# theislab/dca

Hardware: NVIDIA H100
Metric: cells/sec (ZINB AE epoch, device-timed) (higher is better)
Workload: dtype bf16-gemm/f32-acc/f32-loss

## Files before the change

dca_b200/csrc/gene_gemm_tc.cu:

```cuda
#include "engine.h"
#include "tc_common.cuh"

namespace dca {
namespace tc {
int g_gg_profile = 0;
int g_head_bwd_banded = 1;
int g_head_bwd_stagger = 1300;
namespace gg {

constexpr int kThreads = 256;
constexpr uint32_t kZBytes = 128 * 128 * 2;
constexpr uint32_t kWBytes = 64 * 128 * 2;
constexpr uint32_t kHBytes = 128 * 64 * 2;
constexpr uint32_t kOutBytes = 128 * 64 * 4;
constexpr uint32_t kOnesBytes = 16 * 128;
constexpr int kMaxGb = 4;
constexpr int kMaxSlots = 16;

static_assert(kWBytes == kHBytes, "the two item kinds of the banded launch share one stage shape");
template <bool DO_A, bool DO_B, bool BANDED>
constexpr int stages() { return DO_A && DO_B && !BANDED ? 2 : 3; }
template <bool DO_A, bool DO_B, bool BANDED>
constexpr uint32_t stage_bytes() { return BANDED ? kZBytes + kWBytes : kZBytes + (DO_B ? kWBytes : 0) + (DO_A ? kHBytes : 0); }
template <bool DO_A, bool DO_B, bool COLSUM, bool BANDED>
constexpr uint32_t smem_bytes() {
  return stages<DO_A, DO_B, BANDED>() * stage_bytes<DO_A, DO_B, BANDED>() + (DO_A ? kOutBytes : 0) + (COLSUM ? kOnesBytes : 0) + 1024;
}

struct BandItem { int kind, head, gr, gb0, ng, cb0, ncb; };

__host__ __device__ inline BandItem band_item(int k, int n_gb, int n_cb, int gpr, int ranges) {
  const int per_head = n_gb + ranges * n_cb, full_band = gpr + n_cb;
  BandItem it;
  it.head = k / per_head; k -= it.head * per_head;
  it.gr = min(k / full_band, ranges - 1); k -= it.gr * full_band;
  const int gb0 = it.gr * gpr, ng = min(n_gb, gb0 + gpr) - gb0, m = min(ng, n_cb);
  int idx;
  if (k < 2 * m) { it.kind = k & 1; idx = k >> 1; }
  else { it.kind = ng > n_cb ? 0 : 1; idx = k - m; }
  if (it.kind == 0) { it.gb0 = gb0 + idx; it.ng = 1; it.cb0 = 0; it.ncb = n_cb; }
  else { it.gb0 = gb0; it.ng = ng; it.cb0 = idx; it.ncb = 1; }
  return it;
}

struct Params {
  int B, G, n_heads;
  int n_cb, n_gb;
  int gb_per_item, cb_per_item;
  int gene_ranges, cell_splits;
  int total_items;
  int stagger;
  float* db[3];
  float* part; int64_t part_stride;
  const int32_t* rows; const __nv_bfloat16* zsrc; int64_t ldz;
};

__device__ __forceinline__ void cp_async_16(uint32_t smem_dst, const void* src, uint32_t src_bytes) {
  asm volatile("cp.async.cg.shared.global [%0], [%1], 16, %2;" ::"r"(smem_dst), "l"(src), "r"(src_bytes) : "memory");
}
__device__ __forceinline__ void cp_async_commit() { asm volatile("cp.async.commit_group;" ::: "memory"); }
template <int N>
__device__ __forceinline__ void cp_async_wait() { asm volatile("cp.async.wait_group %0;" ::"n"(N) : "memory"); }

template <bool DO_A, bool DO_B, bool COLSUM, bool WK, int MAXG, bool BANDED>
__global__ void __launch_bounds__(kThreads, 1)
gene_gemm_kernel(const __grid_constant__ CUtensorMap map_z0, const __grid_constant__ CUtensorMap map_z1,
                 const __grid_constant__ CUtensorMap map_z2, const __grid_constant__ CUtensorMap map_h,
                 const __grid_constant__ CUtensorMap map_w0, const __grid_constant__ CUtensorMap map_w1,
                 const __grid_constant__ CUtensorMap map_w2, const __grid_constant__ CUtensorMap map_dw0, const __grid_constant__ CUtensorMap map_dw1,
                 const __grid_constant__ CUtensorMap map_dw2, const int dw_transposed, const Params p) {
  static_assert(!BANDED || (DO_A && DO_B && MAXG == 1), "banded items hold one gene block of (a) accumulators");
  constexpr int kStages = stages<DO_A, DO_B, BANDED>();
  constexpr uint32_t kStage = stage_bytes<DO_A, DO_B, BANDED>();
  constexpr uint32_t kHOff = kZBytes + (DO_B && !BANDED ? kWBytes : 0);
  extern __shared__ __align__(1024) uint8_t smem_raw[];
  uint8_t* smem = smem_raw + ((1024u - (smem_u32(smem_raw) & 1023u)) & 1023u);
  uint8_t* s_st = smem;
  float* s_o = reinterpret_cast<float*>(s_st + kStages * kStage);
  uint8_t* s_ones = reinterpret_cast<uint8_t*>(s_o) + (DO_A ? kOutBytes : 0);
  __shared__ uint64_t full[kStages];

  if (threadIdx.x == 0) {
    for (int i = 0; i < kStages; ++i) mbar_init(&full[i], 1);
    fence_barrier_init();
  }
  if (COLSUM) {
    for (int i = threadIdx.x; i < (int)kOnesBytes / 4; i += kThreads) reinterpret_cast<uint32_t*>(s_ones)[i] = 0x3F803F80u;
    fence_proxy_async_smem();
  }
  __syncthreads();

  const int wg = threadIdx.x >> 7, w = (threadIdx.x >> 5) & 3, l = threadIdx.x & 31;
  const int frow = 16 * w + (l >> 2), fcol = 2 * (l & 3);

  auto stage_begin = [&]() {
    if (threadIdx.x == 0) bulk_wait_read<0>();
    __syncthreads();
  };
  auto stage_end = [&](const CUtensorMap* m, int c0, int c1) {
    fence_proxy_async_smem();
    __syncthreads();
    if (threadIdx.x == 0) { tma_reduce_add_2d(m, c0, c1, s_o); bulk_commit(); }
  };

  uint32_t T0 = 0;
  const bool gather = p.rows != nullptr;
  const int g_rh = threadIdx.x >> 3, g_c = threadIdx.x & 7, g_h = g_rh & 1, g_r0 = g_rh >> 1;
  const uint32_t g_dst = g_h * (kZBytes / 2) + g_r0 * 128 + ((g_c ^ (g_r0 & 7)) << 4);
  int src_row[8];
  if constexpr (BANDED) {
    if (p.stagger > 0 && blockIdx.x < p.total_items) {
      const BandItem it = band_item(blockIdx.x, p.n_gb, p.n_cb, p.gb_per_item, p.gene_ranges);
      const long long wait = (long long)(it.kind ? it.cb0 : it.gb0 - it.gr * p.gb_per_item) * p.stagger;
      if (threadIdx.x == 0) {
        const long long c0 = clock64();
        while (clock64() - c0 < wait) __nanosleep(100);
      }
      __syncthreads();
    }
  }
  for (int item = blockIdx.x; item < p.total_items; item += gridDim.x) {
    int head, gr, gb0, ng, cb0, ncb;
    bool ia = DO_A, ib = DO_B;
    if constexpr (BANDED) {
      const BandItem it = band_item(item, p.n_gb, p.n_cb, p.gb_per_item, p.gene_ranges);
      head = it.head; gr = it.gr; gb0 = it.gb0; ng = it.ng; cb0 = it.cb0; ncb = it.ncb;
      ia = it.kind == 0; ib = !ia;
    } else {
      const int cs = item % p.cell_splits, r = item / p.cell_splits;
      gr = r % p.gene_ranges; head = r / p.gene_ranges;
      gb0 = gr * p.gb_per_item; ng = min(p.n_gb, gb0 + p.gb_per_item) - gb0;
      cb0 = cs * p.cb_per_item; ncb = min(p.n_cb, cb0 + p.cb_per_item) - cb0;
    }
    const int n_tiles = ng * ncb;
    const CUtensorMap* mz = head == 0 ? &map_z0 : (head == 1 ? &map_z1 : &map_z2);
    const CUtensorMap* mw = head == 0 ? &map_w0 : (head == 1 ? &map_w1 : &map_w2);
    const CUtensorMap* mdw = head == 0 ? &map_dw0 : (head == 1 ? &map_dw1 : &map_dw2);

    auto issue = [&](int t) {
      const int st = (T0 + t) % kStages;
      const int cb = cb0 + t / ng, gb = gb0 + t % ng;
      uint8_t* dst = s_st + st * kStage;
      mbar_expect_tx(&full[st], gather ? kStage - kZBytes : kStage);
      if (!gather) {
        tma_load_2d(dst, mz, gb * 128, cb * 128, &full[st]);
        tma_load_2d(dst + kZBytes / 2, mz, gb * 128 + 64, cb * 128, &full[st]);
      }
      if (DO_B && ib) {
        if (WK) {
          tma_load_2d(dst + kZBytes, mw, gb * 128, 0, &full[st]);
          tma_load_2d(dst + kZBytes + kWBytes / 2, mw, gb * 128 + 64, 0, &full[st]);
        } else {
          tma_load_2d(dst + kZBytes, mw, 0, gb * 128, &full[st]);
        }
      }
      if (DO_A && ia) tma_load_2d(dst + kHOff, &map_h, 0, cb * 128, &full[st]);
    };
    auto load_rows = [&](int t) {
      const int cb = cb0 + t / ng;
#pragma unroll
      for (int i = 0; i < 8; ++i) {
        const int r = cb * 128 + g_r0 + 16 * i;
        src_row[i] = r < p.B ? __ldg(p.rows + r) : -1;
      }
    };
    auto copy_rows = [&](int t) {
      const int st = (T0 + t) % kStages, g0 = (gb0 + t % ng) * 128 + g_h * 64 + g_c * 8;
      const uint32_t gbytes = g0 < p.G ? (uint32_t)min(16, 2 * (p.G - g0)) : 0u;
      const uint32_t dst = smem_u32(s_st + st * kStage) + g_dst;
#pragma unroll
      for (int i = 0; i < 8; ++i) {
        const bool ok = src_row[i] >= 0 && gbytes != 0;
        cp_async_16(dst + i * 2048, ok ? p.zsrc + (int64_t)src_row[i] * p.ldz + g0 : p.zsrc, ok ? gbytes : 0u);
      }
      if (t + 1 < n_tiles) load_rows(t + 1);
    };
    if (gather) load_rows(0);
    for (int t = 0; t < kStages - 1; ++t) {
      if (t < n_tiles) {
        if (threadIdx.x == 0) issue(t);
        if (gather) copy_rows(t);
      }
      if (gather) cp_async_commit();
    }

    float acc_b[DO_B ? 32 : 1];
    float acc_a[DO_A ? MAXG : 1][32];
    float acc_c[COLSUM ? MAXG : 1][8];
#pragma unroll
    for (int j = 0; j < (DO_A ? MAXG : 1); ++j)
#pragma unroll
      for (int i = 0; i < 32; ++i) acc_a[j][i] = 0.f;
#pragma unroll
    for (int j = 0; j < (COLSUM ? MAXG : 1); ++j)
#pragma unroll
      for (int i = 0; i < 8; ++i) acc_c[j][i] = 0.f;

    int t = 0;
    for (int cbi = 0; cbi < ncb; ++cbi) {
      const int cb = cb0 + cbi;
#pragma unroll
      for (int i = 0; i < (DO_B ? 32 : 1); ++i) acc_b[i] = 0.f;
#pragma unroll
      for (int jj = 0; jj < (DO_A ? MAXG : 1); ++jj)
      for (int j = jj; j < (DO_A && ia ? min(jj + 1, ng) : ng); ++j) {
        if (t + kStages - 1 < n_tiles) {
          if (threadIdx.x == 0) issue(t + kStages - 1);
          if (gather) copy_rows(t + kStages - 1);
        }
        if (gather) {
          cp_async_commit();
          cp_async_wait<kStages - 1>();
          fence_proxy_async_smem();
          __syncthreads();
        }
        const int st = (T0 + t) % kStages;
        mbar_wait(&full[st], ((T0 + t) / kStages) & 1);
        const uint32_t zb = smem_u32(s_st + st * kStage), wb = zb + kZBytes, hb = zb + kHOff;
        wgmma_fence();
        if constexpr (DO_B) {
          if (ib)
#pragma unroll
          for (int h = 0; h < 2; ++h)
#pragma unroll
            for (int k = 0; k < 4; ++k) {
              const uint64_t da = make_smem_desc(zb + h * (kZBytes / 2) + wg * 64 * 128 + k * 32, 0, 1024);
              if (WK) wgmma_m64n64k16<0, 0>(acc_b, da, make_smem_desc(wb + h * (kWBytes / 2) + k * 32, 0, 1024), 1u);
              else wgmma_m64n64k16<0, 1>(acc_b, da, make_smem_desc(wb + (h * 4 + k) * 2048, 0, 1024), 1u);
            }
        }
        if constexpr (DO_A) {
          if (ia)
#pragma unroll
          for (int k = 0; k < 8; ++k) {
            const uint64_t da = make_smem_desc(zb + wg * (kZBytes / 2) + k * 2048, 0, 1024);
            wgmma_m64n64k16<1, 1>(acc_a[jj], da, make_smem_desc(hb + k * 2048, 0, 1024), 1u);
            if constexpr (COLSUM) wgmma_m64n16k16<1, 0>(acc_c[jj], da, make_smem_desc(smem_u32(s_ones) + (k & 3) * 32, 0, 1024), 1u);
          }
        }
        wgmma_commit();
        wgmma_wait<0>();
        if constexpr (DO_B) acc_fence(acc_b);
        if constexpr (DO_A) {
#pragma unroll
          for (int jj2 = 0; jj2 < MAXG; ++jj2) acc_fence(acc_a[jj2]);
        }
        if constexpr (COLSUM) {
#pragma unroll
          for (int jj2 = 0; jj2 < MAXG; ++jj2) acc_fence(acc_c[jj2]);
        }
        __syncthreads();
        ++t;
      }
      if constexpr (DO_B) if (ib) {
        float* dst = p.part + (int64_t)(head * p.gene_ranges + gr) * p.part_stride + (int64_t)cb * 128 * 64;
#pragma unroll
        for (int i = 0; i < 32; i += 2) {
          const int row = wg * 64 + frow + 8 * ((i >> 1) & 1), col = 8 * (i >> 2) + fcol;
          *reinterpret_cast<float2*>(dst + row * 64 + col) = make_float2(acc_b[i], acc_b[i + 1]);
        }
      }
    }
    T0 += n_tiles;
    if (DO_A && ia) {
#pragma unroll
      for (int j = 0; j < MAXG; ++j) {
        if (j >= ng) break;
        const int gb = gb0 + j;
        stage_begin();
        if (dw_transposed) {
#pragma unroll
          for (int i = 0; i < 32; ++i) {
            const int g = wg * 64 + frow + 8 * ((i >> 1) & 1), f = 8 * (i >> 2) + fcol + (i & 1);
            s_o[f * 128 + g] = acc_a[j][i];
          }
          stage_end(mdw, gb * 128, 0);
        } else {
#pragma unroll
          for (int i = 0; i < 32; i += 2) {
            const int g = wg * 64 + frow + 8 * ((i >> 1) & 1), f = 8 * (i >> 2) + fcol;
            *reinterpret_cast<float2*>(s_o + g * 64 + f) = make_float2(acc_a[j][i], acc_a[j][i + 1]);
          }
          stage_end(mdw, 0, gb * 128);
        }
        if constexpr (COLSUM) {
          float* dbh = head == 0 ? p.db[0] : (head == 1 ? p.db[1] : p.db[2]);
          if ((l & 3) == 0 && dbh) {
            const int g = gb * 128 + wg * 64 + frow;
            if (g < p.G) atomicAdd(dbh + g, acc_c[j][0]);
            if (g + 8 < p.G) atomicAdd(dbh + g + 8, acc_c[j][2]);
          }
        }
      }
    }
  }
  if (threadIdx.x == 0) bulk_wait<0>();
}

__global__ void gene_gemm_reduce_kernel(const float* __restrict__ part, int slots, int64_t stride, float* __restrict__ out,
                                        int64_t n) {
  const int64_t i = ((int64_t)blockIdx.x * blockDim.x + threadIdx.x) * 4;
  if (i >= n) return;
  float4 acc = *reinterpret_cast<const float4*>(out + i);
  for (int sl = 0; sl < slots; ++sl) {
    const float4 v = __ldcs(reinterpret_cast<const float4*>(part + sl * stride + i));
    acc.x += v.x; acc.y += v.y; acc.z += v.z; acc.w += v.w;
  }
  *reinterpret_cast<float4*>(out + i) = acc;
}

void plan_a(Params& p, int n_heads, int sm_count) {
  int best_gpi = 1; long long best_cost = -1;
  for (int gpi = 1; gpi <= kMaxGb; ++gpi) {
    const long long items = (long long)cdiv(p.n_gb, gpi) * n_heads, rounds = (items + sm_count - 1) / sm_count;
    const long long cost = rounds * ((long long)gpi * p.n_cb + 2ll * gpi);
    if (best_cost < 0 || cost < best_cost) { best_cost = cost; best_gpi = gpi; }
  }
  p.gb_per_item = best_gpi; p.gene_ranges = cdiv(p.n_gb, best_gpi);
  p.cb_per_item = p.n_cb; p.cell_splits = 1;
  p.total_items = p.gene_ranges * n_heads;
}
void plan_b(Params& p, int n_heads, int sm_count) {
  p.cb_per_item = 1; p.cell_splits = p.n_cb;
  int gsplits = cdiv(4 * sm_count, p.n_cb * n_heads); if (gsplits < 1) gsplits = 1;
  if (gsplits > kMaxSlots / n_heads) gsplits = kMaxSlots / n_heads;
  if (gsplits > p.n_gb) gsplits = p.n_gb;
  while (gsplits > 1 && cdiv(p.n_gb, gsplits) < 4) --gsplits;
  p.gb_per_item = cdiv(p.n_gb, gsplits); p.gene_ranges = cdiv(p.n_gb, p.gb_per_item);
  p.total_items = p.gene_ranges * p.cell_splits * n_heads;
}
void plan_banded(Params& p, int n_heads, int sm_count, int* grid) {
  plan_b(p, n_heads, sm_count);
  p.total_items = n_heads * (p.n_gb + p.gene_ranges * p.n_cb);
  const int band = p.gb_per_item + p.n_cb;
  *grid = min(p.total_items, sm_count >= band ? sm_count / band * band : sm_count);
}

}

size_t gene_gemm_workspace_bytes(int B) { return sizeof(float) * (size_t)gg::kMaxSlots * cdiv(B, 128) * 128 * 64; }

int gene_gemm_tc(int mode, const __nv_bfloat16* const Z[3], int64_t ldz, const int32_t* rows, int B, int G, int n_heads,
                 const __nv_bfloat16* H, const __nv_bfloat16* const W[3], float* out_b, float* const dW[3], int64_t dW_ld,
                 int dW_transposed, float* const db[3], void* ws, size_t ws_bytes, int sm_count, cudaStream_t s) {
  using namespace gg;
  if (ldz % 8 != 0) { set_error("gene_gemm_tc: ldz must be a multiple of 8 (16-byte TMA stride)"); return DCA_ERR_BAD_ARG; }
  if (mode < 1 || mode > 3) { set_error("gene_gemm_tc: bad mode %d", mode); return DCA_ERR_BAD_ARG; }
  if (rows && (mode == 3 || n_heads != 1)) { set_error("gene_gemm_tc: row indices are for modes 1 and 2 (one Z)"); return DCA_ERR_BAD_ARG; }
  const bool do_a = mode & 2, do_b = mode & 1;
  if (do_b && (!ws || ws_bytes < gene_gemm_workspace_bytes(B))) { set_error("gene_gemm_tc: workspace too small"); return DCA_ERR_BAD_ARG; }
  CUtensorMap mz[3], mh, mw[3], mdw[3];
  for (int i = 0; i < 3; ++i) DCA_TRY(make_tensor_map_2d(&mz[i], Z[i < n_heads ? i : 0], 2, 1, (uint64_t)B, (uint64_t)G, (uint64_t)ldz, 128, 64, 1));
  mh = mz[0];
  for (int i = 0; i < 3; ++i) mw[i] = mdw[i] = mz[0];
  if (do_a) {
    DCA_TRY(make_tensor_map_2d(&mh, H, 2, 1, (uint64_t)B, 64, 64, 128, 64, 1));
    for (int i = 0; i < 3; ++i) {
      float* d = dW[i < n_heads ? i : 0];
      if (dW_transposed) DCA_TRY(make_tensor_map_2d(&mdw[i], d, 4, 0, 64, (uint64_t)G, (uint64_t)dW_ld, 64, 128, 0));
      else {
        if (dW_ld != 64) { set_error("gene_gemm_tc: non-transposed dW needs ld == 64"); return DCA_ERR_BAD_ARG; }
        DCA_TRY(make_tensor_map_2d(&mdw[i], d, 4, 0, (uint64_t)G, 64, 64, 128, 64, 0));
      }
    }
  }
  if (do_b) {
    for (int i = 0; i < 3; ++i) {
      const __nv_bfloat16* w = W[i < n_heads ? i : 0];
      if (mode == 3) DCA_TRY(make_tensor_map_2d(&mw[i], w, 2, 1, 64, (uint64_t)G, (uint64_t)G, 64, 64, 1));
      else DCA_TRY(make_tensor_map_2d(&mw[i], w, 2, 1, (uint64_t)G, 64, 64, 128, 64, 1));
    }
  }
  Params base{};
  base.B = B; base.G = G; base.n_heads = n_heads;
  base.n_cb = cdiv(B, 128); base.n_gb = cdiv(G, 128);
  for (int i = 0; i < 3; ++i) base.db[i] = db ? db[i] : nullptr;
  base.part = reinterpret_cast<float*>(ws); base.part_stride = (int64_t)base.n_cb * 128 * 64;
  base.rows = rows; base.zsrc = Z[0]; base.ldz = ldz;

#define DCA_GG_LAUNCH(P, GRID, A, Bb, Cc, WKk, MG, BND)                                                                \
  do {                                                                                                                 \
    static bool attr = false;                                                                                          \
    constexpr uint32_t sm = smem_bytes<A, Bb, Cc, BND>();                                                              \
    if (!attr) { DCA_CUDA_OK(cudaFuncSetAttribute(gene_gemm_kernel<A, Bb, Cc, WKk, MG, BND>, cudaFuncAttributeMaxDynamicSharedMemorySize, (int)sm)); attr = true; } \
    gene_gemm_kernel<A, Bb, Cc, WKk, MG, BND><<<GRID, kThreads, sm, s>>>(mz[0], mz[1], mz[2], mh, mw[0], mw[1], mw[2],  \
                                                                          mdw[0], mdw[1], mdw[2], dW_transposed, P);  \
    DCA_LAUNCH_CHECK();                                                                                                \
  } while (0)

  if (mode == 3 && g_head_bwd_banded) {
    Params p = base;
    int grid = 0;
    plan_banded(p, n_heads, sm_count, &grid);
    p.stagger = g_head_bwd_stagger;
    DCA_GG_LAUNCH(p, grid, true, true, true, true, 1, true);
    const int64_t n = (int64_t)B * 64;
    gene_gemm_reduce_kernel<<<(unsigned)cdiv(n / 4, 256), 256, 0, s>>>(p.part, p.gene_ranges * n_heads, p.part_stride, out_b, n);
    DCA_LAUNCH_CHECK();
    return DCA_OK;
  }
  if (do_a) {
    Params p = base;
    plan_a(p, n_heads, sm_count);
    const int grid = min(p.total_items, sm_count);
    if (mode == 3) DCA_GG_LAUNCH(p, grid, true, false, true, false, kMaxGb, false);
    else DCA_GG_LAUNCH(p, grid, true, false, false, false, kMaxGb, false);
  }
  if (do_b) {
    Params p = base;
    plan_b(p, n_heads, sm_count);
    const int grid = min(p.total_items, sm_count);
    if (mode == 3) DCA_GG_LAUNCH(p, grid, false, true, false, true, 1, false);
    else DCA_GG_LAUNCH(p, grid, false, true, false, false, 1, false);
    const int64_t n = (int64_t)B * 64;
    gene_gemm_reduce_kernel<<<(unsigned)cdiv(n / 4, 256), 256, 0, s>>>(p.part, p.gene_ranges * n_heads, p.part_stride, out_b, n);
    DCA_LAUNCH_CHECK();
  }
#undef DCA_GG_LAUNCH
  return DCA_OK;
}

}
}

using namespace dca;
extern "C" int dca_tc_gene_gemm_rows(int32_t mode, const void* Z0, const void* Z1, const void* Z2, int64_t ldz,
                                     const int32_t* rows, int32_t batch, int32_t genes, int32_t n_heads, const void* H,
                                     const void* W, float* out_b, float* dW0, float* dW1, float* dW2, int64_t dW_ld,
                                     int32_t dW_transposed, float* db0, float* db1, float* db2, void* stream, int32_t sm_count) {
  if (!Z0 || batch <= 0 || genes <= 0 || n_heads < 1 || n_heads > 3) { set_error("dca_tc_gene_gemm: bad argument"); return DCA_ERR_BAD_ARG; }
  int dev = 0, sms = 132;
  cudaGetDevice(&dev);
  cudaDeviceGetAttribute(&sms, cudaDevAttrMultiProcessorCount, dev);
  if (sm_count > 0 && sm_count < sms) sms = sm_count;
  const __nv_bfloat16* Z[3] = {(const __nv_bfloat16*)Z0, (const __nv_bfloat16*)Z1, (const __nv_bfloat16*)Z2};
  float* dW[3] = {dW0, dW1, dW2};
  float* db[3] = {db0, db1, db2};
  const __nv_bfloat16* Wp[3];
  for (int i = 0; i < 3; ++i) Wp[i] = (const __nv_bfloat16*)W + (mode == 3 ? (size_t)(i < n_heads ? i : 0) * 64 * genes : 0);
  cudaStream_t st = (cudaStream_t)stream;
  const size_t ws_bytes = tc::gene_gemm_workspace_bytes(batch);
  void* ws = nullptr;
  DCA_CUDA_OK(cudaMallocAsync(&ws, ws_bytes, st));
  const int rc = tc::gene_gemm_tc(mode, Z, ldz, rows, batch, genes, n_heads, (const __nv_bfloat16*)H, Wp, out_b, dW,
                                  dW_ld, dW_transposed, db, ws, ws_bytes, sms, st);
  DCA_CUDA_OK(cudaFreeAsync(ws, st));
  return rc;
}
extern "C" int dca_tc_gene_gemm_sms(int32_t mode, const void* Z0, const void* Z1, const void* Z2, int64_t ldz,
                                    int32_t batch, int32_t genes, int32_t n_heads, const void* H, const void* W, float* out_b,
                                    float* dW0, float* dW1, float* dW2, int64_t dW_ld, int32_t dW_transposed, float* db0,
                                    float* db1, float* db2, void* stream, int32_t sm_count) {
  return dca_tc_gene_gemm_rows(mode, Z0, Z1, Z2, ldz, nullptr, batch, genes, n_heads, H, W, out_b, dW0, dW1, dW2, dW_ld,
                               dW_transposed, db0, db1, db2, stream, sm_count);
}
extern "C" int dca_tc_gene_gemm(int32_t mode, const void* Z0, const void* Z1, const void* Z2, int64_t ldz, int32_t batch,
                                int32_t genes, int32_t n_heads, const void* H, const void* W, float* out_b, float* dW0,
                                float* dW1, float* dW2, int64_t dW_ld, int32_t dW_transposed, float* db0, float* db1,
                                float* db2, void* stream) {
  return dca_tc_gene_gemm_sms(mode, Z0, Z1, Z2, ldz, batch, genes, n_heads, H, W, out_b, dW0, dW1, dW2, dW_ld,
                              dW_transposed, db0, db1, db2, stream, 0);
}
extern "C" int dca_head_bwd_schedule(int32_t batch, int32_t genes, int32_t n_heads, int32_t sm_count, int32_t banded,
                                     int32_t* items, int64_t cap, int64_t* n_items, int32_t* grid) {
  if (batch <= 0 || genes <= 0 || n_heads < 1 || n_heads > 3 || sm_count < 1 || !n_items || !grid) {
    set_error("dca_head_bwd_schedule: bad argument"); return DCA_ERR_BAD_ARG;
  }
  tc::gg::Params base{};
  base.n_cb = cdiv(batch, 128); base.n_gb = cdiv(genes, 128);
  int64_t k = 0;
  auto put = [&](int launch, int kind, int head, int gb0, int ng, int cb0, int ncb, int slot) {
    if (items && k < cap) {
      int32_t* r = items + 8 * k;
      r[0] = launch; r[1] = kind; r[2] = head; r[3] = gb0; r[4] = ng; r[5] = cb0; r[6] = ncb; r[7] = slot;
    }
    ++k;
  };
  if (banded) {
    tc::gg::Params p = base;
    plan_banded(p, n_heads, sm_count, &grid[0]);
    grid[1] = 0;
    for (int i = 0; i < p.total_items; ++i) {
      const tc::gg::BandItem it = tc::gg::band_item(i, p.n_gb, p.n_cb, p.gb_per_item, p.gene_ranges);
      put(0, it.kind, it.head, it.gb0, it.ng, it.cb0, it.ncb, it.kind ? it.head * p.gene_ranges + it.gr : -1);
    }
  } else {
    tc::gg::Params pa = base, pb = base;
    plan_a(pa, n_heads, sm_count);
    plan_b(pb, n_heads, sm_count);
    grid[0] = std::min(pa.total_items, (int)sm_count); grid[1] = std::min(pb.total_items, (int)sm_count);
    for (int pass = 0; pass < 2; ++pass) {
      const tc::gg::Params& p = pass ? pb : pa;
      for (int i = 0; i < p.total_items; ++i) {
        const int cs = i % p.cell_splits, r = i / p.cell_splits, gr = r % p.gene_ranges, head = r / p.gene_ranges;
        const int gb0 = gr * p.gb_per_item, cb0 = cs * p.cb_per_item;
        put(pass, pass, head, gb0, std::min(p.n_gb, gb0 + p.gb_per_item) - gb0, cb0, std::min(p.n_cb, cb0 + p.cb_per_item) - cb0,
            pass ? head * p.gene_ranges + gr : -1);
      }
    }
  }
  *n_items = k;
  return DCA_OK;
}
```

dca_b200/csrc/zinb_loss.cu:

```cuda
#include "dca_internal.cuh"
#include <string>
#include "zinb_math.cuh"
#include "tc_common.cuh"
#include "head_act.cuh"
#include <cstdlib>

namespace dca {
namespace tc { extern int g_gg_profile; extern int g_head_bwd_banded; extern int g_head_bwd_stagger; }

namespace {

constexpr int kThreads = 256;
constexpr int kVec = 4;
constexpr int kColsPerBlock = kThreads * kVec;
constexpr int kMaxBlocks = 65536;

struct LossTune { int target_blocks; unsigned producer_sleep_ns, consumer_sleep_ns; int branch_free; int ring; };
LossTune g_tune = {0 , 0u, 0u, 1 ,
                   1 };

int sm_count_cached() {
  static int n = 0;
  if (!n) { int dev = 0; if (cudaGetDevice(&dev) != cudaSuccess || cudaDeviceGetAttribute(&n, cudaDevAttrMultiProcessorCount, dev) != cudaSuccess || n <= 0) n = 132; }
  return n;
}

struct Plan { int col_blocks, rows_per_block, row_chunks; };

inline Plan make_plan(int B, int G, int cols_per_block, int max_rpb = 1 << 30) {
  Plan p;
  p.col_blocks = cdiv(G, cols_per_block);
  const int target = g_tune.target_blocks > 0 ? g_tune.target_blocks
                     : ((long long)B * G <= (32ll << 20) ? 3 * sm_count_cached() : 16 * sm_count_cached());
  int chunks = target / p.col_blocks;
  if (chunks < 1) chunks = 1;
  if (chunks > B) chunks = B;
  int rpb = cdiv(B, chunks);
  if (rpb < 2 && B >= 2) rpb = 2;
  if (rpb > max_rpb) rpb = max_rpb;
  while ((long long)cdiv(B, rpb) * p.col_blocks > kMaxBlocks && rpb < max_rpb) ++rpb;
  p.rows_per_block = rpb;
  p.row_chunks = cdiv(B, rpb);
  return p;
}

__device__ __forceinline__ float4 ld4(const float* p) { return *reinterpret_cast<const float4*>(p); }
__device__ __forceinline__ float4 ld4_stream(const float* p) {
  float4 r;
  asm volatile("ld.global.nc.L1::no_allocate.v4.f32 {%0,%1,%2,%3}, [%4];"
               : "=f"(r.x), "=f"(r.y), "=f"(r.z), "=f"(r.w) : "l"(p));
  return r;
}
__device__ __forceinline__ void st4(float* p, float a, float b, float c, float d) {
  *reinterpret_cast<float4*>(p) = make_float4(a, b, c, d);
}
__device__ __forceinline__ void st4(__nv_bfloat16* p, float a, float b, float c, float d) {
  __nv_bfloat162 lo = __floats2bfloat162_rn(a, b), hi = __floats2bfloat162_rn(c, d);
  uint2 v;
  v.x = *reinterpret_cast<uint32_t*>(&lo);
  v.y = *reinterpret_cast<uint32_t*>(&hi);
  *reinterpret_cast<uint2*>(p) = v;
}
__device__ __forceinline__ void st1(float* p, float a) { *p = a; }
__device__ __forceinline__ void st1(__nv_bfloat16* p, float a) { *p = __float2bfloat16_rn(a); }

__device__ __forceinline__ double block_reduce_sum(float v, double* smem ) {
  double d = (double)v;
#pragma unroll
  for (int o = 16; o > 0; o >>= 1) d += __shfl_xor_sync(0xffffffffu, d, o);
  const int w = threadIdx.x >> 5, l = threadIdx.x & 31;
  if (l == 0) smem[w] = d;
  __syncthreads();
  double t = 0.0;
  if (w == 0) {
    t = (l < (kThreads >> 5)) ? smem[l] : 0.0;
#pragma unroll
    for (int o = 4; o > 0; o >>= 1) t += __shfl_xor_sync(0xffffffffu, t, o);
  }
  return t;
}

template <int VEC>
struct RowVals { float y[VEC], m[VEC], d[VEC], p[VEC]; float sf; };

template <bool HAS_PI, bool COND_DISP, int VEC>
__device__ __forceinline__ void load_row(RowVals<VEC>& v, const float* __restrict__ Y, int64_t ldy,
                                         const int32_t* __restrict__ rows, const float* __restrict__ sf,
                                         const float* m, const float* d, const float* pi, int64_t ld, int r, int col0) {
  const int64_t yr = rows ? (int64_t)rows[r] : (int64_t)r;
  v.sf = sf ? sf[yr] : 1.0f;
  const float* yp = Y + yr * ldy + col0;
  const int64_t off = (int64_t)r * ld + col0;
  if (VEC == 4) {
    float4 t = ld4_stream(yp); v.y[0] = t.x; v.y[1] = t.y; v.y[2] = t.z; v.y[3] = t.w;
    t = ld4(m + off); v.m[0] = t.x; v.m[1] = t.y; v.m[2] = t.z; v.m[3] = t.w;
    if (COND_DISP) { t = ld4(d + off); v.d[0] = t.x; v.d[1] = t.y; v.d[2] = t.z; v.d[3] = t.w; }
    if (HAS_PI) { t = ld4(pi + off); v.p[0] = t.x; v.p[1] = t.y; v.p[2] = t.z; v.p[3] = t.w; }
  } else {
    v.y[0] = yp[0]; v.m[0] = m[off];
    if (COND_DISP) v.d[0] = d[off];
    if (HAS_PI) v.p[0] = pi[off];
  }
}

template <bool HAS_PI, bool COND_DISP, typename GT, int VEC, bool BWD>
__global__ void __launch_bounds__(kThreads)
zinb_loss_kernel(const float* __restrict__ Y, int64_t ldy, const int32_t* __restrict__ rows,
                 const float* __restrict__ sf, const float* m, const float* d, const float* pi,
                 int64_t ld, int B, int G, float ridge, float inv_n, int rows_per_block,
                 GT* dzm, GT* dzd, GT* dzp, float* __restrict__ dth_partial,
                 double* __restrict__ loss_partial, const float* __restrict__ lf_global) {
  __shared__ double red[8];
  __shared__ float lf[zmath::kLogFactN];
  if (threadIdx.x < zmath::kLogFactN) lf[threadIdx.x] = lf_global[threadIdx.x];
  __syncthreads();
  using Ops = zmath::FastOps;
  const int col0 = (blockIdx.x * kThreads + threadIdx.x) * VEC;
  const int r0 = blockIdx.y * rows_per_block;
  const int r1 = min(B, r0 + rows_per_block);
  float lsum = 0.f;
  float tacc[VEC];
#pragma unroll
  for (int j = 0; j < VEC; ++j) tacc[j] = 0.f;

  if (col0 < G) {
    float thg[VEC];
    if (!COND_DISP) {
#pragma unroll
      for (int j = 0; j < VEC; ++j) thg[j] = (col0 + j < G) ? d[col0 + j] : 1.f;
    }
    RowVals<VEC> cur, nxt;
    load_row<HAS_PI, COND_DISP, VEC>(cur, Y, ldy, rows, sf, m, d, pi, ld, r0, col0);
    for (int r = r0; r < r1; ++r) {
      if (r + 1 < r1) load_row<HAS_PI, COND_DISP, VEC>(nxt, Y, ldy, rows, sf, m, d, pi, ld, r + 1, col0);
      const int64_t off = (int64_t)r * ld + col0;
      float gm[VEC], gd[VEC], gp[VEC];
#pragma unroll
      for (int j = 0; j < VEC; ++j) {
        const float th = COND_DISP ? cur.d[j] : thg[j];
        const float p = HAS_PI ? cur.p[j] : 0.f;
        if (BWD) {
          zmath::Elem e = zmath::zinb_elem<Ops, HAS_PI, COND_DISP>(cur.y[j], cur.m[j], cur.sf, th, p, ridge, lf);
          lsum += e.loss;
          gm[j] = e.gm * inv_n; gd[j] = e.gd * inv_n; gp[j] = e.gp * inv_n;
          if (!COND_DISP) tacc[j] += e.gd;
        } else {
          lsum += zmath::zinb_elem_loss<Ops, HAS_PI>(cur.y[j], cur.m[j], cur.sf, th, p, ridge, lf);
        }
      }
      if (BWD) {
        if (VEC == 4) {
          st4(dzm + off, gm[0], gm[1], gm[2], gm[3]);
          if (COND_DISP) st4(dzd + off, gd[0], gd[1], gd[2], gd[3]);
          if (HAS_PI) st4(dzp + off, gp[0], gp[1], gp[2], gp[3]);
        } else {
          st1(dzm + off, gm[0]);
          if (COND_DISP) st1(dzd + off, gd[0]);
          if (HAS_PI) st1(dzp + off, gp[0]);
        }
      }
      cur = nxt;
// ... 842 lines not shown
  if (!a.ws || a.ws_bytes < need) { set_error("zinb_loss: workspace too small (%zu < %zu)", a.ws_bytes, need); return DCA_ERR_BAD_ARG; }
  double* lpart = reinterpret_cast<double*>(a.ws);
  auto al16 = [](const void* q) { return (reinterpret_cast<uintptr_t>(q) & 15) == 0; };
  bool vec = (a.G % 4 == 0) && (a.ld % 4 == 0) && (a.ldy % 4 == 0) && al16(a.Y) && al16(a.m) && (!cond || al16(a.d)) &&
             (!has_pi || al16(a.pi));
  if (BWD) vec = vec && al16(a.dzm) && (!cond || al16(a.dzd)) && (!has_pi || al16(a.dzp));
  const Plan p = make_plan(a.B, a.G, vec ? kColsPerBlock : kThreads);
  dim3 grid(p.col_blocks, p.row_chunks), block(kThreads);
  float* tpart = a.dtheta;
  if (BWD && !cond) DCA_CUDA_OK(cudaMemsetAsync(a.dtheta, 0, sizeof(float) * (size_t)a.G, s));

  static const bool use_compact = [] { const char* e = getenv("DCA_LOSS_KERNEL"); return e && e[0] == 'c'; }();
  const Plan ps = make_plan(a.B, a.G, kColsPerBlock, kMaxRowsPerBlock);
  const bool staged_ok = BWD && vec && has_pi && !use_compact && (long long)ps.row_chunks * ps.col_blocks <= kMaxBlocks &&
                         ps.row_chunks <= 65535;
  if (staged_ok) {
    grid = dim3(ps.col_blocks, ps.row_chunks);
    FoldArgs fa{reinterpret_cast<unsigned*>(reinterpret_cast<char*>(a.ws) + sizeof(double) * (size_t)kMaxBlocks), a.loss_sum,
                a.fin_penalty, a.fin_loss_slot, a.fin_epoch_acc, a.fin_batch};
    if (!a.counter_ready) DCA_CUDA_OK(cudaMemsetAsync(fa.counter, 0, sizeof(unsigned), s));
#define DCA_RING2(CD, GT, IQ)                                                                                     \
  do {                                                                                                             \
    constexpr size_t sm = IQ ? (size_t)(kRing + 1) * (CD ? 4 : 3) * kColsPerBlock * 4 + (size_t)(kThreads / 32) * 32 * kVec     \
                             : (size_t)kRing * (CD ? 4 : 3) * kColsPerBlock * 4 + (size_t)(kThreads / 32) * 32 * kVec * 16; \
    static bool attr = false;                                                                                      \
    if (!attr) { DCA_CUDA_OK(cudaFuncSetAttribute(zinb_loss_bwd_ring_kernel<CD, GT, IQ>, cudaFuncAttributeMaxDynamicSharedMemorySize, (int)sm)); attr = true; } \
    zinb_loss_bwd_ring_kernel<CD, GT, IQ><<<grid, kThreads, sm, s>>>(a.Y, a.ldy, a.rows, a.sf, a.m, a.d, a.pi, a.ld, a.B, a.G, a.ridge, \
        a.inv_n, ps.rows_per_block, (GT*)a.dzm, (GT*)a.dzd, (GT*)a.dzp, tpart, lpart, lf_dev, fa);                  \
  } while (0)
#define DCA_RING(CD, GT) do { if (g_tune.ring == 2) DCA_RING2(CD, GT, true); else DCA_RING2(CD, GT, false); } while (0)
    if (g_tune.ring) {
      if (a.grad_bf16) { if (cond) DCA_RING(true, __nv_bfloat16); else DCA_RING(false, __nv_bfloat16); }
      else             { if (cond) DCA_RING(true, float); else DCA_RING(false, float); }
      DCA_LAUNCH_CHECK();
      return DCA_OK;
    }
#undef DCA_RING
#undef DCA_RING2
#define DCA_STAGED2(CD, GT, BFV)                                                                                   \
  do {                                                                                                             \
    constexpr size_t sm = (size_t)kStageRows * (CD ? 4 : 3) * kColsPerBlock * 4 + (size_t)(kThreads / 32) * 32 * kVec * 16; \
    static bool attr = false;                                                                                      \
    if (!attr) { DCA_CUDA_OK(cudaFuncSetAttribute(zinb_loss_bwd_staged_kernel<CD, GT, BFV>, cudaFuncAttributeMaxDynamicSharedMemorySize, (int)sm)); attr = true; } \
    zinb_loss_bwd_staged_kernel<CD, GT, BFV><<<grid, kStagedThreads, sm, s>>>(a.Y, a.ldy, a.rows, a.sf, a.m, a.d, a.pi, a.ld, a.B, \
        a.G, a.ridge, a.inv_n, ps.rows_per_block, (GT*)a.dzm, (GT*)a.dzd, (GT*)a.dzp, tpart, lpart, lf_dev, fa,     \
        g_tune.producer_sleep_ns, g_tune.consumer_sleep_ns);                                                       \
  } while (0)
#define DCA_STAGED(CD, GT) do { if (g_tune.branch_free) DCA_STAGED2(CD, GT, true); else DCA_STAGED2(CD, GT, false); } while (0)
    if (a.grad_bf16) { if (cond) DCA_STAGED(true, __nv_bfloat16); else DCA_STAGED(false, __nv_bfloat16); }
    else             { if (cond) DCA_STAGED(true, float); else DCA_STAGED(false, float); }
#undef DCA_STAGED2
#undef DCA_STAGED
    DCA_LAUNCH_CHECK();
    return DCA_OK;
  } else if (BWD && vec && has_pi) {
#define DCA_COMPACT(CD, GT)                                                                                   \
  zinb_loss_bwd_compact_kernel<CD, GT><<<grid, block, 0, s>>>(a.Y, a.ldy, a.rows, a.sf, a.m, a.d, a.pi, a.ld, a.B, a.G, \
                                                              a.ridge, a.inv_n, p.rows_per_block, (GT*)a.dzm,  \
                                                              (GT*)a.dzd, (GT*)a.dzp, tpart, lpart, lf_dev)
    if (a.grad_bf16) { if (cond) DCA_COMPACT(true, __nv_bfloat16); else DCA_COMPACT(false, __nv_bfloat16); }
    else             { if (cond) DCA_COMPACT(true, float); else DCA_COMPACT(false, float); }
#undef DCA_COMPACT
  } else {
#define DCA_LOSS_LAUNCH(HP, CD, GT, V)                                                                 \
  zinb_loss_kernel<HP, CD, GT, V, BWD><<<grid, block, 0, s>>>(                                          \
      a.Y, a.ldy, a.rows, a.sf, a.m, a.d, a.pi, a.ld, a.B, a.G, a.ridge, a.inv_n, p.rows_per_block,      \
      (GT*)a.dzm, (GT*)a.dzd, (GT*)a.dzp, tpart, lpart, lf_dev)
#define DCA_LOSS_DISPATCH(GT, V)                                   \
  do {                                                             \
    if (has_pi && cond) DCA_LOSS_LAUNCH(true, true, GT, V);        \
    else if (has_pi && !cond) DCA_LOSS_LAUNCH(true, false, GT, V); \
    else if (!has_pi && cond) DCA_LOSS_LAUNCH(false, true, GT, V); \
    else DCA_LOSS_LAUNCH(false, false, GT, V);                     \
  } while (0)
    if (BWD && a.grad_bf16) {
      if (vec) DCA_LOSS_DISPATCH(__nv_bfloat16, 4); else DCA_LOSS_DISPATCH(__nv_bfloat16, 1);
    } else {
      if (vec) DCA_LOSS_DISPATCH(float, 4); else DCA_LOSS_DISPATCH(float, 1);
    }
#undef DCA_LOSS_DISPATCH
#undef DCA_LOSS_LAUNCH
  }
  DCA_LAUNCH_CHECK();
  fold_partials_kernel<<<1, 256, 0, s>>>(lpart, (int)(grid.x * grid.y), a.loss_sum, BWD ? 0 : 1, a.fin_penalty, a.inv_n,
                                         a.fin_batch, BWD ? a.fin_loss_slot : nullptr, a.fin_epoch_acc);
  DCA_LAUNCH_CHECK();
  return DCA_OK;
}

}

const float* loss_log_fact_table() { return log_fact_table_device(); }
int g_fused_heads_default = 0;

size_t loss_workspace_bytes(int B, int G) {
  (void)B; (void)G;
  return sizeof(double) * (size_t)kMaxBlocks + 256;
}

int zinb_loss_fwd_bwd(const LossArgs& a, cudaStream_t s) { return launch<true>(a, s); }
int zinb_loss_fwd(const LossArgs& a, cudaStream_t s) { return launch<false>(a, s); }

int heads_loss_tc(const HeadsLossArgs& a, cudaStream_t s) {
  using namespace hl;
  const int B = a.B, G = a.G;
  auto al = [](const void* q, uintptr_t n) { return (reinterpret_cast<uintptr_t>(q) & (n - 1)) == 0; };
  if (B <= 0 || G <= 0 || G % 8 != 0 || a.ldy % 4 != 0 || !al(a.Y, 16) || a.ldz % 4 != 0 || a.ldz < G ||
      !al(a.dz[0], 8) || !al(a.dz[1], 8) || !al(a.dz[2], 8)) {
    set_error("heads_loss_tc: need G %% 8 == 0, a 16-byte aligned Y with ldy %% 4 == 0 and 8-byte aligned dZ with ldz %% 4 == 0 (>= G)");
    return DCA_ERR_BAD_ARG;
  }
  const float* lf_dev = log_fact_table_device();
  if (!lf_dev) return DCA_ERR_CUDA;
  if (!a.ws || a.ws_bytes < loss_workspace_bytes(B, G)) { set_error("heads_loss_tc: workspace too small"); return DCA_ERR_BAD_ARG; }
  CUtensorMap mh, mw[3];
  DCA_TRY(tc::make_tensor_map_2d(&mh, a.H3, 2, 1, (uint64_t)B, 64, 64, 64, 64, 1));
  for (int i = 0; i < 3; ++i) DCA_TRY(tc::make_tensor_map_2d(&mw[i], a.W[i], 2, 1, 64, (uint64_t)G, (uint64_t)G, 64, 64, 1));
  Params p;
  for (int i = 0; i < 3; ++i) { p.bias[i] = a.bias[i]; p.dz[i] = a.dz[i]; }
  p.Y = a.Y; p.ldy = a.ldy; p.rows = a.rows; p.sf = a.sf; p.B = B; p.G = G; p.ldz = a.ldz;
  p.nblk = cdiv(B, 64);
  const long long units = (long long)cdiv(G, 128) * p.nblk;
  if (units > INT_MAX) { set_error("heads_loss_tc: %lld (gene tile, cell block) units, over 2^31 - 1", units); return DCA_ERR_BAD_ARG; }
  p.units = (int)units;
  p.ridge = a.ridge; p.inv_n = a.inv_n;
  p.loss_partial = reinterpret_cast<double*>(a.ws); p.lf = lf_dev;
  FoldArgs fa{reinterpret_cast<unsigned*>(reinterpret_cast<char*>(a.ws) + sizeof(double) * (size_t)kMaxBlocks), a.loss_sum,
              a.fin_penalty, a.fin_loss_slot, a.fin_epoch_acc, a.fin_batch};
  if (!a.counter_ready) DCA_CUDA_OK(cudaMemsetAsync(fa.counter, 0, sizeof(unsigned), s));
  static bool attr = false;
  if (!attr) { DCA_CUDA_OK(cudaFuncSetAttribute(heads_loss_kernel, cudaFuncAttributeMaxDynamicSharedMemorySize, (int)kSmemBytes)); attr = true; }
  const int grid = (int)std::min<long long>(p.units, sm_count_cached());
  heads_loss_kernel<<<grid, kCtaThreads, kSmemBytes, s>>>(mh, mw[0], mw[1], mw[2], p, fa);
  DCA_LAUNCH_CHECK();
  return DCA_OK;
}

}

using namespace dca;

extern "C" int dca_set_tunable(const char* name, int64_t value) {
  if (!name) { set_error("dca_set_tunable: null name"); return DCA_ERR_BAD_ARG; }
  const std::string n(name);
  if (n == "loss_target_blocks" && value >= 0 && value <= kMaxBlocks) g_tune.target_blocks = (int)value;
  else if (n == "loss_producer_sleep_ns" && value >= 0 && value <= 100000) g_tune.producer_sleep_ns = (unsigned)value;
  else if (n == "loss_consumer_sleep_ns" && value >= 0 && value <= 100000) g_tune.consumer_sleep_ns = (unsigned)value;
  else if (n == "fused_heads" && (value == 0 || value == 1)) g_fused_heads_default = (int)value;
  else if (n == "loss_branch_free" && (value == 0 || value == 1)) g_tune.branch_free = (int)value;
  else if (n == "loss_ring" && value >= 0 && value <= 2) g_tune.ring = (int)value;
  else if (n == "gg_profile" && (value == 0 || value == 1)) tc::g_gg_profile = (int)value;
  else if (n == "head_bwd_banded" && (value == 0 || value == 1)) tc::g_head_bwd_banded = (int)value;
  else if (n == "head_bwd_stagger" && value >= 0 && value <= 100000) tc::g_head_bwd_stagger = (int)value;
  else { set_error("dca_set_tunable: unknown name or value out of range (%s = %lld)", name, (long long)value); return DCA_ERR_BAD_ARG; }
  return DCA_OK;
}

extern "C" int dca_zinb_loss_workspace_bytes(int32_t batch, int32_t genes, size_t* bytes) {
  if (!bytes || batch <= 0 || genes <= 0) { set_error("dca_zinb_loss_workspace_bytes: bad argument"); return DCA_ERR_BAD_ARG; }
  *bytes = loss_workspace_bytes(batch, genes);
  return DCA_OK;
}

extern "C" int dca_zinb_loss_fwd_bwd(const float* Y, int64_t ldy, const int32_t* rows, const float* sf,
                                     const float* m, const float* d, const float* pi, int64_t ld,
                                     int32_t batch, int32_t genes, int32_t ae_type, float ridge, float inv_n,
                                     void* dzm, void* dzd, void* dzp, int32_t grad_dtype, float* dtheta,
                                     double* loss_sum, void* workspace, size_t workspace_bytes, void* stream) {
  if (ae_type < 0 || ae_type > 3) { set_error("dca_zinb_loss_fwd_bwd: unknown ae_type %d", ae_type); return DCA_ERR_BAD_ARG; }
  LossArgs a{Y, ldy, rows, sf, m, d, pi, ld, batch, genes, ae_type, ridge, inv_n, dzm, dzd, dzp,
             grad_dtype == DCA_BF16 ? 1 : 0, dtheta, loss_sum, workspace, workspace_bytes};
  return zinb_loss_fwd_bwd(a, (cudaStream_t)stream);
}

extern "C" int dca_tc_heads_loss(const void* Hb, int32_t batch, const void* Wk, const float* bias, int32_t genes,
                                 const float* Y, int64_t ldy, const int32_t* rows, const float* sf, float ridge, float inv_n,
                                 void* dzm, void* dzd, void* dzp, int64_t ldz, double* loss_sum, void* workspace,
                                 size_t workspace_bytes, void* stream) {
  if (!Hb || !Wk || !bias || !Y || !dzm || !dzd || !dzp || !loss_sum || batch <= 0 || genes <= 0) {
    set_error("dca_tc_heads_loss: bad argument"); return DCA_ERR_BAD_ARG;
  }
  HeadsLossArgs a{};
  a.H3 = (const __nv_bfloat16*)Hb; a.B = batch; a.G = genes;
  for (int i = 0; i < 3; ++i) { a.W[i] = (const __nv_bfloat16*)Wk + (size_t)i * 64 * genes; a.bias[i] = bias + (size_t)i * genes; }
  a.Y = Y; a.ldy = ldy; a.rows = rows; a.sf = sf; a.ridge = ridge; a.inv_n = inv_n;
  a.dz[0] = (__nv_bfloat16*)dzm; a.dz[1] = (__nv_bfloat16*)dzd; a.dz[2] = (__nv_bfloat16*)dzp; a.ldz = ldz;
  a.loss_sum = loss_sum; a.ws = workspace; a.ws_bytes = workspace_bytes;
  return heads_loss_tc(a, (cudaStream_t)stream);
}

extern "C" int dca_zinb_loss_fwd(const float* Y, int64_t ldy, const int32_t* rows, const float* sf,
                                 const float* m, const float* d, const float* pi, int64_t ld, int32_t batch,
                                 int32_t genes, int32_t ae_type, float ridge, double* loss_sum, void* workspace,
                                 size_t workspace_bytes, void* stream) {
  if (ae_type < 0 || ae_type > 3) { set_error("dca_zinb_loss_fwd: unknown ae_type %d", ae_type); return DCA_ERR_BAD_ARG; }
  LossArgs a{Y, ldy, rows, sf, m, d, pi, ld, batch, genes, ae_type, ridge, 1.0f, nullptr, nullptr, nullptr,
             0, nullptr, loss_sum, workspace, workspace_bytes};
  return zinb_loss_fwd(a, (cudaStream_t)stream);
}

extern "C" int dca_zinb_elem_host(int32_t ae_type, float y, float m, float sf, float d, float pi, float ridge,
                                  float out[4]) {
  zmath::Elem e;
  static float lf[zmath::kLogFactN];
  static bool lf_ready = false;
  if (!lf_ready) { zmath::fill_log_fact(lf); lf_ready = true; }
  using P = zmath::PreciseOps;
  if (ae_type & 0x200) {
    const int base = ae_type & 0xff;
    if (base != DCA_AE_ZINB_CONDDISP && base != DCA_AE_ZINB) { set_error("dca_zinb_elem_host: kernel variant needs a ZINB type"); return DCA_ERR_BAD_ARG; }
    const bool cd = base == DCA_AE_ZINB_CONDDISP;
    const float2 m2 = zmath::splat(m), d2 = zmath::splat(d), p2 = zmath::splat(pi), mu2 = zmath::mul2(m2, zmath::splat(sf));
    const zmath::Fin2 f = cd ? zmath::finish_factors_pair<P, true>(m2, d2, p2, 1.0f) : zmath::finish_factors_pair<P, false>(m2, d2, p2, 1.0f);
    float loss, gmu, dth, dpi;
    if (y < 1e-8f) {
      const zmath::Raw2 z = zmath::zinb_zero_pair<P>(mu2, d2, p2);
      loss = -zmath::kLn2 * z.lgD.y; gmu = z.gmu.y; dth = z.dth.y; dpi = z.dpi.y;
    } else {
      const zmath::Raw1 r = zmath::zinb_nb_raw<P>(y, mu2.x, d, pi, lf);
      loss = r.loss; gmu = r.gmu; dth = r.dth; dpi = r.dpi;
    }
    if (ridge != 0.f) { loss += ridge * pi * pi; dpi = fmaf(2.0f * ridge, pi, dpi); }
    out[0] = loss; out[1] = gmu * f.fm.y; out[2] = dth * f.fd.y; out[3] = dpi * f.fp.y;
    return DCA_OK;
  }
  if (ae_type & 0x100) {
    const int base = ae_type & 0xff;
    if (base != DCA_AE_ZINB_CONDDISP && base != DCA_AE_ZINB) { set_error("dca_zinb_elem_host: kernel variant needs a ZINB type"); return DCA_ERR_BAD_ARG; }
    if (y < 1e-8f) {
      e = base == DCA_AE_ZINB_CONDDISP ? zmath::zinb_elem_zero_bf<P, true>(m, sf, d, pi, ridge)
                                       : zmath::zinb_elem_zero_bf<P, false>(m, sf, d, pi, ridge);
    } else if (base == DCA_AE_ZINB_CONDDISP) {
      e = zmath::zinb_elem_nb_mu<P>(y, m * sf, d, pi, ridge, lf);
      if (!(m > 1e-5f && m < 1e6f)) e.gm = 0.f;
    } else {
      e = zmath::zinb_elem<P, true, false>(y, m, sf, d, pi, ridge, lf);
    }
    out[0] = e.loss; out[1] = e.gm; out[2] = e.gd; out[3] = e.gp;
    return DCA_OK;
  }
  switch (ae_type) {
    case DCA_AE_ZINB_CONDDISP: e = zmath::zinb_elem<P, true, true>(y, m, sf, d, pi, ridge, lf); break;
    case DCA_AE_ZINB: e = zmath::zinb_elem<P, true, false>(y, m, sf, d, pi, ridge, lf); break;
    case DCA_AE_NB_CONDDISP: e = zmath::zinb_elem<P, false, true>(y, m, sf, d, pi, ridge, lf); break;
    case DCA_AE_NB: e = zmath::zinb_elem<P, false, false>(y, m, sf, d, pi, ridge, lf); break;
    default: set_error("dca_zinb_elem_host: unknown ae_type %d", ae_type); return DCA_ERR_BAD_ARG;
  }
  out[0] = e.loss; out[1] = e.gm; out[2] = e.gd; out[3] = e.gp;
  return DCA_OK;
}
```

Baseline: 3.097 million.

## Add wide-gene encoder backward kernel and longer cell items for encoder forward

```diff
diff --git a/dca_b200/csrc/gene_gemm_tc.cu b/dca_b200/csrc/gene_gemm_tc.cu
--- a/dca_b200/csrc/gene_gemm_tc.cu
+++ b/dca_b200/csrc/gene_gemm_tc.cu
@@ -6,6 +6,8 @@
 int g_gg_profile = 0;
 int g_head_bwd_banded = 1;
 int g_head_bwd_stagger = 1300;
+int g_enc_fwd_long_items = 1;
+int g_enc_bwd_wide = 1;
 namespace gg {
 
 constexpr int kThreads = 256;
@@ -307,6 +309,102 @@
     acc.x += v.x; acc.y += v.y; acc.z += v.z; acc.w += v.w;
   }
   *reinterpret_cast<float4*>(out + i) = acc;
+}
+
+namespace wide {
+constexpr int kWg = 3, kThreads = 128 * kWg, kStages = 3, kGenes = 64 * kWg;
+constexpr uint32_t kBoxBytes = 128 * 64 * 2;
+constexpr uint32_t kZBytes = kWg * kBoxBytes;
+constexpr uint32_t kStage = kZBytes + kHBytes;
+constexpr uint32_t kSmem = kStages * kStage + 1024;
+static_assert(kGenes * 64 * 4 <= kStages * kStage, "the flush staging fits in the stage ring");
+}
+
+__global__ void __launch_bounds__(wide::kThreads, 1)
+enc_bwd_wide_kernel(const __grid_constant__ CUtensorMap map_h, const __grid_constant__ CUtensorMap map_dw, const Params p) {
+  constexpr int kWg = wide::kWg, kStages = wide::kStages, kGenes = wide::kGenes;
+  constexpr uint32_t kBoxBytes = wide::kBoxBytes, kZBytes = wide::kZBytes, kStage = wide::kStage;
+  extern __shared__ __align__(1024) uint8_t smem_raw[];
+  uint8_t* s_st = smem_raw + ((1024u - (smem_u32(smem_raw) & 1023u)) & 1023u);
+  float* s_o = reinterpret_cast<float*>(s_st);
+  __shared__ uint64_t full[kStages];
+  if (threadIdx.x == 0) {
+    for (int i = 0; i < kStages; ++i) mbar_init(&full[i], 1);
+    fence_barrier_init();
+  }
+  __syncthreads();
+  const int wg = threadIdx.x >> 7, w = (threadIdx.x >> 5) & 3, l = threadIdx.x & 31;
+  const int frow = 16 * w + (l >> 2), fcol = 2 * (l & 3);
+  const int g_pair = threadIdx.x >> 3, g_c = threadIdx.x & 7, g_box = g_pair % kWg, g_r0 = g_pair / kWg;
+  const uint32_t g_dst = g_box * kBoxBytes + g_r0 * 128 + ((g_c ^ (g_r0 & 7)) << 4);
+  uint32_t T0 = 0;
+  int src_row[8];
+  for (int item = blockIdx.x; item < p.total_items; item += gridDim.x) {
+    if (item != (int)blockIdx.x) {
+      if (threadIdx.x == 0) bulk_wait_read<0>();
+      __syncthreads();
+    }
+    const int g0 = item * kGenes + g_box * 64 + g_c * 8;
+    const uint32_t gbytes = g0 < p.G ? (uint32_t)min(16, 2 * (p.G - g0)) : 0u;
+    auto load_rows = [&](int cb) {
+#pragma unroll
+      for (int i = 0; i < 8; ++i) {
+        const int r = cb * 128 + g_r0 + 16 * i;
+        src_row[i] = r < p.B ? (p.rows ? __ldg(p.rows + r) : r) : -1;
+      }
+    };
+    auto issue = [&](int t) {
+      const int st = (T0 + t) % kStages;
+      uint8_t* dst = s_st + st * kStage;
+      if (threadIdx.x == 0) {
+        mbar_expect_tx(&full[st], kHBytes);
+        tma_load_2d(dst + kZBytes, &map_h, 0, t * 128, &full[st]);
+      }
+      const uint32_t d = smem_u32(dst) + g_dst;
+#pragma unroll
+      for (int i = 0; i < 8; ++i) {
+        const bool ok = src_row[i] >= 0 && gbytes != 0;
+        cp_async_16(d + i * 2048, ok ? p.zsrc + (int64_t)src_row[i] * p.ldz + g0 : p.zsrc, ok ? gbytes : 0u);
+      }
+      if (t + 1 < p.n_cb) load_rows(t + 1);
+    };
+    load_rows(0);
+    for (int t = 0; t < kStages - 1; ++t) {
+      if (t < p.n_cb) issue(t);
+      cp_async_commit();
+    }
+    float acc[32];
+#pragma unroll
+    for (int i = 0; i < 32; ++i) acc[i] = 0.f;
+    for (int t = 0; t < p.n_cb; ++t) {
+      if (t + kStages - 1 < p.n_cb) issue(t + kStages - 1);
+      cp_async_commit();
+      cp_async_wait<kStages - 1>();
+      fence_proxy_async_smem();
+      __syncthreads();
+      const int st = (T0 + t) % kStages;
+      mbar_wait(&full[st], ((T0 + t) / kStages) & 1);
+      const uint32_t zb = smem_u32(s_st + st * kStage), hb = zb + kZBytes;
+      wgmma_fence();
+#pragma unroll
+      for (int k = 0; k < 8; ++k)
+        wgmma_m64n64k16<1, 1>(acc, make_smem_desc(zb + wg * kBoxBytes + k * 2048, 0, 1024), make_smem_desc(hb + k * 2048, 0, 1024), 1u);
+      wgmma_commit();
+      wgmma_wait<0>();
+      acc_fence(acc);
+      __syncthreads();
+    }
+    T0 += p.n_cb;
+#pragma unroll
+    for (int i = 0; i < 32; i += 2) {
+      const int g = wg * 64 + frow + 8 * ((i >> 1) & 1), f = 8 * (i >> 2) + fcol;
+      *reinterpret_cast<float2*>(s_o + g * 64 + f) = make_float2(acc[i], acc[i + 1]);
+    }
+    fence_proxy_async_smem();
+    __syncthreads();
+    if (threadIdx.x == 0) { tma_reduce_add_2d(&map_dw, 0, item * kGenes, s_o); bulk_commit(); }
+  }
+  if (threadIdx.x == 0) bulk_wait<0>();
 }
 
 void plan_a(Params& p, int n_heads, int sm_count) {
@@ -388,14 +486,28 @@
     DCA_LAUNCH_CHECK();                                                                                                \
   } while (0)
 
+  auto add_slots = [&](const Params& p) -> int {
+    const int64_t n = (int64_t)B * 64;
+    gene_gemm_reduce_kernel<<<(unsigned)cdiv(n / 4, 256), 256, 0, s>>>(p.part, p.gene_ranges * n_heads, p.part_stride, out_b, n);
+    DCA_LAUNCH_CHECK();
+    return DCA_OK;
+  };
   if (mode == 3 && g_head_bwd_banded) {
     Params p = base;
     int grid = 0;
     plan_banded(p, n_heads, sm_count, &grid);
     p.stagger = g_head_bwd_stagger;
     DCA_GG_LAUNCH(p, grid, true, true, true, true, 1, true);
-    const int64_t n = (int64_t)B * 64;
-    gene_gemm_reduce_kernel<<<(unsigned)cdiv(n / 4, 256), 256, 0, s>>>(p.part, p.gene_ranges * n_heads, p.part_stride, out_b, n);
+    return add_slots(p);
+  }
+  if (mode == 2 && g_enc_bwd_wide && !dW_transposed) {
+    Params p = base;
+    p.total_items = cdiv(G, wide::kGenes);
+    CUtensorMap mdw_wide;
+    DCA_TRY(make_tensor_map_2d(&mdw_wide, dW[0], 4, 0, (uint64_t)G, 64, 64, wide::kGenes, 64, 0));
+    static bool attr = false;
+    if (!attr) { DCA_CUDA_OK(cudaFuncSetAttribute(enc_bwd_wide_kernel, cudaFuncAttributeMaxDynamicSharedMemorySize, (int)wide::kSmem)); attr = true; }
+    enc_bwd_wide_kernel<<<min(p.total_items, sm_count), wide::kThreads, wide::kSmem, s>>>(mh, mdw_wide, p);
     DCA_LAUNCH_CHECK();
     return DCA_OK;
   }
@@ -409,12 +521,15 @@
   if (do_b) {
     Params p = base;
     plan_b(p, n_heads, sm_count);
+    if (mode == 1 && g_enc_fwd_long_items) {
+      p.cb_per_item = min(p.n_cb, cdiv(p.n_cb * p.gene_ranges * n_heads, sm_count));
+      p.cell_splits = cdiv(p.n_cb, p.cb_per_item);
+      p.total_items = p.gene_ranges * p.cell_splits * n_heads;
+    }
     const int grid = min(p.total_items, sm_count);
     if (mode == 3) DCA_GG_LAUNCH(p, grid, false, true, false, true, 1, false);
     else DCA_GG_LAUNCH(p, grid, false, true, false, false, 1, false);
-    const int64_t n = (int64_t)B * 64;
-    gene_gemm_reduce_kernel<<<(unsigned)cdiv(n / 4, 256), 256, 0, s>>>(p.part, p.gene_ranges * n_heads, p.part_stride, out_b, n);
-    DCA_LAUNCH_CHECK();
+    DCA_TRY(add_slots(p));
   }
 #undef DCA_GG_LAUNCH
   return DCA_OK;
diff --git a/dca_b200/csrc/zinb_loss.cu b/dca_b200/csrc/zinb_loss.cu
--- a/dca_b200/csrc/zinb_loss.cu
+++ b/dca_b200/csrc/zinb_loss.cu
@@ -6,7 +6,8 @@
 #include <cstdlib>
 
 namespace dca {
-namespace tc { extern int g_gg_profile; extern int g_head_bwd_banded; extern int g_head_bwd_stagger; }
+namespace tc { extern int g_gg_profile; extern int g_head_bwd_banded; extern int g_head_bwd_stagger; extern int g_enc_fwd_long_items;
+               extern int g_enc_bwd_wide; }
 
 namespace {
 
@@ -1155,6 +1156,8 @@
   else if (n == "gg_profile" && (value == 0 || value == 1)) tc::g_gg_profile = (int)value;
   else if (n == "head_bwd_banded" && (value == 0 || value == 1)) tc::g_head_bwd_banded = (int)value;
   else if (n == "head_bwd_stagger" && value >= 0 && value <= 100000) tc::g_head_bwd_stagger = (int)value;
+  else if (n == "enc_fwd_long_items" && (value == 0 || value == 1)) tc::g_enc_fwd_long_items = (int)value;
+  else if (n == "enc_bwd_wide" && (value == 0 || value == 1)) tc::g_enc_bwd_wide = (int)value;
   else { set_error("dca_set_tunable: unknown name or value out of range (%s = %lld)", name, (long long)value); return DCA_ERR_BAD_ARG; }
   return DCA_OK;
 }
```

Result: faster. 3.193 million, median of 6 (+3.1%).
